# HKU-BAL/MegaPath-Nano

Hardware: AMD Instinct MI355X
Metric: Gbp/min ONT reads aligned+species-assigned vs RefSeq, 1/2/4/8 MI355X (higher is better)
Workload: dtype int32

## Files before the change

include/mpn_map.h:

```cpp
#ifndef MPN_MAP_H
#define MPN_MAP_H
#include <stdint.h>

#ifdef __cplusplus
extern "C" {
#endif

typedef struct mpn_index mpn_index;

typedef struct {
    int32_t k, w;
    float mid_occ_frac;
    int32_t mid_occ;
    int32_t max_gap, bw, max_chain_skip, max_chain_iter, min_cnt, min_chain_score;
    float mask_level, pri_ratio;
    int32_t best_n;
    int32_t max_join_long, max_join_short, min_join_flank_sc;
    float min_join_flank_ratio;
    int32_t a, b, q, e, q2, e2, sc_ambi, zdrop, zdrop_inv, end_bonus, min_dp_max, min_ksw_len;
    float max_clip_ratio;
    int64_t max_sw_mat;
    int32_t with_cigar;
    uint32_t seed;
    int32_t host_threads;
// ... 23 lines not shown
int32_t mpn_index_part_info(const char *path, int64_t offset, int64_t *bases, int64_t *next_offset);
int32_t mpn_index_n_seq(const mpn_index *idx);
int32_t mpn_index_seq_len(const mpn_index *idx, int32_t i);
int32_t mpn_index_seq_name(const mpn_index *idx, int32_t i, char *buf, int32_t cap);
int32_t mpn_index_k(const mpn_index *idx);
int32_t mpn_index_w(const mpn_index *idx);
int64_t mpn_index_n_minimizers(const mpn_index *idx);
int64_t mpn_index_n_keys(const mpn_index *idx);
int32_t mpn_index_mid_occ(const mpn_index *idx, float frac);
int64_t mpn_index_fetch_seq(const mpn_index *idx, int32_t i, int64_t start, int64_t len, char *out);
int mpn_index_export(const mpn_index *idx, uint64_t *keys, int64_t *key_off, uint64_t *pos);

int64_t mpn_sketch_batch(int32_t n, const char *seqs, const int64_t *seq_off, const int32_t *seq_len, int32_t k,
                         int32_t w, int64_t *mz_off, uint64_t *mz, int64_t cap);

int mpn_seed_chain_batch(const mpn_index *idx, const mpn_map_opt *opt, int32_t n, const char *seqs,
                         const int64_t *seq_off, const int32_t *seq_len, int64_t *n_anchor, int32_t *rep_len,
                         int64_t *chain_off, uint64_t *u, int64_t u_cap, int64_t *anchor_off, uint64_t *b,
                         int64_t b_cap);

int mpn_chain_batch(const mpn_map_opt *opt, int32_t n, const int64_t *anchor_off, const uint64_t *anchors, int32_t chain_item,
                    int32_t bt_par_min, int32_t grid_cap, int32_t *n_chain, int64_t *n_chained, uint64_t *u, int64_t *recs,
                    int64_t u_cap, uint64_t *b, int64_t b_cap);

int mpn_seed_anchors_batch(int32_t k, int32_t n_seq, const int32_t *lens, int64_t n_keys, const uint64_t *keys, const int64_t *key_off,
                           const uint64_t *pos, const mpn_map_opt *opt, int32_t n, const int64_t *mz_off, const uint64_t *mz,
                           const int32_t *seq_len, int64_t flt_round2, int32_t flt_wgs, int32_t grid_cap, int64_t *n_anchor, int32_t *rep_len,
                           int64_t *span_sum, int64_t *anchor_off, uint64_t *anchors, int64_t cap, int64_t counts[4]);

int mpn_ext_dp_batch(const mpn_map_opt *opt, int32_t n, const uint8_t *qcodes, const int64_t *q_off, const int32_t *q_len,
                     const uint8_t *tcodes, const int64_t *t_off, const int32_t *t_len, const int32_t *w, const int32_t *zdrop,
                     const int32_t *end_bonus, const int32_t *flag, int32_t force_kernel, int32_t *out9, uint32_t *cigar_pool,
                     int64_t cigar_cap, int64_t *cig_off);

int mpn_aln_tags_batch(int32_t n, const uint8_t *qcodes, const int64_t *q_off, const int32_t *q_len,
                       const int32_t *qs, const int32_t *qe, const int32_t *rev,
                       const uint8_t *tcodes, const int64_t *t_off, const int32_t *t_len, const int32_t *ts,
                       const uint32_t *cigar, const int64_t *cig_off, const int32_t *n_cigar, int32_t out_tags,
                       char *cs, int64_t cs_cap, int64_t *cs_off, char *md, int64_t md_cap, int64_t *md_off,
                       uint32_t *eqx, int64_t eqx_cap, int64_t *eqx_off);

int mpn_aln_finish_batch(const mpn_map_opt *opt, int32_t n, const uint8_t *qcodes, const int64_t *q_off, const int32_t *q_len,
                         const int32_t *qs, const int32_t *qe, const int32_t *rev,
                         const uint8_t *tcodes, const int64_t *t_off, const int32_t *t_len, const int32_t *ts,
                         const uint32_t *cigar, const int64_t *cig_off, const int32_t *n_cigar, int32_t force_class,
                         int32_t *out8, uint32_t *cigar_out);
// ... 68 lines not shown
```

megapath_nano_amd/csrc/map_kernels.h:

```cpp
#pragma once
#include "mpn_common.h"
#include "map_types.h"

#include <type_traits>

namespace mpn {

__device__ __forceinline__ uint64_t hash64m(uint64_t key, uint64_t mask) {
    key = (~key + (key << 21)) & mask;
    key = key ^ key >> 24;
    key = ((key + (key << 3)) + (key << 8)) & mask;
    key = key ^ key >> 14;
    key = ((key + (key << 2)) + (key << 4)) & mask;
    key = key ^ key >> 28;
    key = (key + (key << 31)) & mask;
    return key;
}

constexpr int SKETCH_FAST_MAX_W = 32;

template <bool HASH64>
__device__ __forceinline__ uint64_t sketch_hash(uint64_t key, uint64_t mask) {
    if (HASH64) return hash64m(key, mask);
    uint32_t h = (uint32_t)key;
// ... 1405 lines not shown
                }
                const uint32_t rank = __popcll(same & ((1ULL << lane) - 1));
                if (act && rank == 0) wcnt[wv][dg] = __popcll(same);
                __syncthreads();
                if (act) {
                    uint32_t o = bins[dg] + rank;
                    for (int w2 = 0; w2 < wv; ++w2) o += wcnt[w2][dg];
                    dst[o] = r;
                }
                __syncthreads();
                bins[tid] += wcnt[0][tid] + wcnt[1][tid] + wcnt[2][tid] + wcnt[3][tid];
                __syncthreads();
            }
            uint64_t *sw = src; src = dst; dst = sw;
            __threadfence_block();
            __syncthreads();
        }
        if (src != U + base) for (int i = tid; i < n; i += 256) U[base + i] = src[i];
        __syncthreads();
    }
}

constexpr int BT_PAR_MIN = 16;

__global__ __launch_bounds__(64) void chain_backtrack_kernel(const u128 *__restrict__ anchors, const int64_t *__restrict__ anchor_off,
                                                             int n_reads, ChainParams cp, const int32_t *__restrict__ F,
                                                             const int32_t *__restrict__ P, int32_t *__restrict__ T,
                                                             int32_t *__restrict__ V, uint64_t *__restrict__ U,
                                                             const int32_t *__restrict__ n_ends, u128 *__restrict__ B,
                                                             uint64_t *__restrict__ Uc, unsigned long long *__restrict__ used,
                                                             int64_t *__restrict__ u_pos, int64_t *__restrict__ b_pos,
                                                             int32_t *__restrict__ n_chain, int64_t *__restrict__ n_chained,
                                                             ChainRec *__restrict__ Rc, int par_min) {
    __shared__ int s_k;
    __shared__ unsigned long long s_up, s_bp;
    const int lane = threadIdx.x;
    for (int read = blockIdx.x; read < n_reads; read += gridDim.x) {
        const int64_t base = anchor_off[read];
        const int64_t n = anchor_off[read + 1] - base;
        const u128 *a = anchors + base;
        const int32_t *f = F + base, *p = P + base;
        int32_t *t = T + base, *v = V + base;
        uint64_t *u = U + base;
        const int n_u = n_ends[read];
        if (n_u >= par_min) {
            for (int64_t i = lane; i < n; i += 64) t[i] = 0x7fffffff;
            __builtin_amdgcn_fence(__ATOMIC_RELEASE, "agent");
            __syncthreads();
            for (int e0 = 0; e0 < n_u; e0 += 64) {
                const int e = e0 + lane;
                if (e < n_u) {
                    int32_t j = (int32_t)u[e];
                    while (j >= 0) { const int32_t nj = p[j]; if (atomicMin(&t[j], e) < e) break; j = nj; }
                }
            }
            __builtin_amdgcn_fence(__ATOMIC_ACQ_REL, "agent");
            __syncthreads();
            int k_run = 0, nv_run = 0;
            for (int e0 = 0; e0 < n_u; e0 += 64) {
                const int e = e0 + lane;
                int cnt = 0;
                if (e < n_u) {
                    const uint64_t ui = u[e];
                    int32_t j = p[(int32_t)ui];
                    cnt = 1;
                    while (j >= 0) { const int32_t tj = t[j], nj = p[j]; if (tj != e) break; ++cnt; j = nj; }
                    const bool keep = cnt >= cp.min_cnt && (j < 0 || (int32_t)(ui >> 32) - f[j] >= cp.min_sc);
                    if (!keep) cnt = 0;
// ... 90 lines not shown
            for (int j = lane; j < ni; j += 64) {
                const u128 cur = a[v[off + (ni - j - 1)]];
                b[off + j] = cur;
                const int span = (int)(cur.y >> 32 & 0xff);
                if (j == 0) { ml += span; bl += span; }
                else {
                    const u128 prev = a[v[off + (ni - j)]];
                    const int tl = (int32_t)cur.x - (int32_t)prev.x, ql = (int32_t)cur.y - (int32_t)prev.y;
                    bl += tl > ql ? tl : ql;
                    ml += tl > span && ql > span ? span : tl < ql ? tl : ql;
                }
            }
            ml = __builtin_amdgcn_readlane(wave_scan_add(ml), 63);
            bl = __builtin_amdgcn_readlane(wave_scan_add(bl), 63);
            if (lane == 0) {
                const u128 first = a[v[off + ni - 1]], last = a[v[off]];
                rc[c] = ChainRec{first.x, first.y, last.x, last.y, ml, bl};
            }
            off += ni;
        }
        for (int c = lane; c < k; c += 64) uc[c] = u[c];
        __syncthreads();
    }
}

__global__ __launch_bounds__(256) void idx_bucket_hist_kernel(const u128 *__restrict__ mz, int64_t n, int shift, unsigned long long *__restrict__ hist) {
    for (int64_t i = (int64_t)blockIdx.x * blockDim.x + threadIdx.x; i < n; i += (int64_t)gridDim.x * blockDim.x)
        atomicAdd(&hist[(mz[i].x >> 8) >> shift], 1ULL);
}

__global__ __launch_bounds__(256) void idx_bucket_scatter_kernel(const u128 *__restrict__ mz, int64_t n, int shift,
                                                                 unsigned long long *__restrict__ cursor, u128 *__restrict__ out) {
    for (int64_t i = (int64_t)blockIdx.x * blockDim.x + threadIdx.x; i < n; i += (int64_t)gridDim.x * blockDim.x) {
        u128 r = mz[i];
        r.x >>= 8;
        const unsigned long long p = atomicAdd(&cursor[r.x >> shift], 1ULL);
        out[p] = r;
    }
}

__global__ __launch_bounds__(256) void idx_flag_count_kernel(const u128 *__restrict__ rec, int64_t n, int64_t *__restrict__ block_cnt) {
    __shared__ int s[256];
    const int64_t base = (int64_t)blockIdx.x * 2048;
    int c = 0;
    for (int k = 0; k < 8; ++k) {
        const int64_t i = base + k * 256 + threadIdx.x;
// ... 89 lines not shown
```

megapath_nano_amd/csrc/mapper.hip:

```cpp
#include "map_kernels.h"
#include "mapper_internal.h"
#include "stage_input.h"
#include "../../include/mpn_map.h"

#include <algorithm>
#include <memory>
#include <mutex>
#include <string.h>
#include <time.h>
#include <sys/stat.h>
#include <string>
#include <vector>

namespace mpn {

hipError_t stream_sync(hipStream_t st) {
    struct Ev {
        hipEvent_t e = nullptr;
        ~Ev() { if (e) (void)hipEventDestroy(e); }
    };
    static thread_local Ev ev;
    hipError_t rc;
    if (!ev.e && (rc = hipEventCreateWithFlags(&ev.e, hipEventDisableTiming)) != hipSuccess) return rc;
    if ((rc = hipEventRecord(ev.e, st)) != hipSuccess) return rc;
// ... 189 lines not shown
}

int sketch_reads(int k, int w, int n, const uint8_t *d_seqs, const int64_t *d_off, const int32_t *d_len, const int32_t *h_len, ReadSketch &sk,
                 StreamLease &st) {
    EvTimer ev(st);
    sk.valid = false;
    if (sketch_device(d_seqs, d_off, d_len, h_len, n, k, w, 0, sk.mz_off, sk.mz, &sk.n_mz, st, &ev)) return -1;
    MPN_HIP_CHECK(stream_sync(st));
    ev.resolve();
    sk.k = k; sk.w = w; sk.valid = true;
    return 0;
}

static int chain_gap_check(const mpn_map_opt *opt, const char *who) {
    if (opt->max_gap > CHAIN_MAX_GAP) {
        set_error("%s: max_gap %d is beyond %d, the largest the chain DP's 32-bit ring coordinate holds", who, opt->max_gap, CHAIN_MAX_GAP);
        return -1;
    }
    return 0;
}

static int alloc_chain_tables(SeedChainOut &o, int n) {
    const size_t N = (size_t)n, o1 = (N + 1) * 8, o2 = o1 + N * 8, o3 = o2 + N * 8, o4 = o3 + N * 8, o5 = o4 + N * 4, o6 = (o5 + N * 4 + 7) & ~(size_t)7;
    o.tables_bytes = o6 + (size_t)(2 + WORK_SLOTS) * 8;
    if (o.tables.alloc(o.tables_bytes)) return -1;
    auto view = [&](auto &buf, size_t off, size_t count) { buf.release(); buf.p = reinterpret_cast<decltype(buf.p)>(o.tables.p + off); buf.n = count; buf.owned = false; };
    view(o.n_anchor, 0, N + 1); view(o.n_chained, o1, N); view(o.u_pos, o2, N); view(o.b_pos, o3, N);
    view(o.n_chain, o4, N); view(o.rep_len, o5, N); view(o.used, o6, 2 + WORK_SLOTS);
    return 0;
}

struct ChainKnobs {
    int chain_item = 0;
    int bt_par_min = 0;
    int grid_cap = 0;
};
struct ChainScratch {
    DevBuf<int64_t> kept, piece_kept, piece_off;
    DevBuf<float> avg_qspan;
    DevBuf<int32_t> F, P, T, V;
    DevBuf<uint64_t> Utmp;
    DevBuf<ChainSeg> seg_big, seg_small;
};
static int chain_enqueue(const mpn_map_opt *opt, int n, int64_t n_a, SeedChainOut &o, u128 *tmp, unsigned long long *read_kept,
                         const unsigned long long *span_sum, unsigned int *seg_counters, const ChainKnobs &kn, ChainScratch &cs, StreamLease &st,
                         EvTimer &ev) {
    auto &[kept, piece_kept, piece_off, avg_qspan, F, P, T, V, Utmp, seg_big, seg_small] = cs;
    ChainParams cp;
    cp.max_dist_x = opt->max_gap; cp.max_dist_y = opt->max_gap; cp.bw = opt->bw; cp.max_skip = opt->max_chain_skip;
    cp.max_iter = opt->max_chain_iter; cp.min_cnt = opt->min_cnt; cp.min_sc = opt->min_chain_score;
    const auto capped = [&](int64_t grid) { return (int)(kn.grid_cap > 0 ? std::min<int64_t>(grid, kn.grid_cap) : grid); };
    const int g = capped(std::max(1, std::min(n, 256 * 32)));
    const int64_t n_pieces = (n_a + COMPACT_PIECE - 1) / COMPACT_PIECE;
    if (kept.alloc((size_t)n + 1) || o.c_off.alloc((size_t)n + 1) || avg_qspan.alloc(n) || piece_kept.alloc((size_t)n_pieces + 1) ||
        piece_off.alloc((size_t)n_pieces + 1))
        return -1;
    const int gp = capped(std::max<int64_t>(1, std::min<int64_t>(n_pieces, 256 * 64)));
    if (n_a > 0) {
// ... 17 lines not shown
                           cp.max_dist_x, cp.min_cnt, (int64_t *)nullptr, (unsigned long long *)nullptr, (const int64_t *)piece_off.p, ca);
        MPN_HIP_CHECK(hipGetLastError());
    }
    ev.mark(46);
    static const int chain_item_env = []() { const char *e = getenv("MPN_CHAIN_ITEM"); return e ? std::min(CHAIN_BIG, std::max(16, atoi(e))) : CHAIN_ITEM; }();
    const int chain_item = kn.chain_item > 0 ? std::min(CHAIN_BIG, std::max(16, kn.chain_item)) : chain_item_env;
    if (seg_big.alloc((size_t)n_c / CHAIN_BIG + (size_t)n + 1) || seg_small.alloc((size_t)n_c / chain_item + (size_t)n + 1)) return -1;
    hipLaunchKernelGGL(chain_segments_kernel, dim3(g), dim3(64), 0, st, (const u128 *)ca, (const int64_t *)o.c_off.p, n, cp, avg_qspan.p, 1, seg_big.p,
                       seg_small.p, seg_counters, chain_item);
    MPN_HIP_CHECK(hipGetLastError());
    ev.mark(13);
    hipLaunchKernelGGL(chain_dp_kernel, dim3(capped(256 * 32)), dim3(64), 0, st, (const u128 *)ca, (const int64_t *)o.c_off.p, (const float *)avg_qspan.p,
                       (const ChainSeg *)seg_big.p, (const ChainSeg *)seg_small.p, seg_counters, cp, F.p, P.p, T.p, V.p);
    MPN_HIP_CHECK(hipGetLastError());
    ev.mark(13, 37);
    hipLaunchKernelGGL(chain_ends_kernel, dim3(g), dim3(64), 0, st, (const int64_t *)o.c_off.p, n, cp, F.p, P.p, T.p, V.p, o.u.p, o.n_ends.p);
    MPN_HIP_CHECK(hipGetLastError());
    hipLaunchKernelGGL(chain_sort_ends_kernel, dim3(capped(std::max(1, std::min(n, 256 * 8)))), dim3(256), 0, st, o.u.p, Utmp.p,
                       (const int64_t *)o.c_off.p, o.n_ends.p, n);
    MPN_HIP_CHECK(hipGetLastError());
    o.u_compact.p = Utmp.p; o.u_compact.n = Utmp.n; o.u_compact.owned = Utmp.owned; Utmp.p = nullptr; Utmp.n = 0;
    static const int bt_par_min_env = []() { const char *e = getenv("MPN_BT_PAR_MIN"); return e ? std::max(1, atoi(e)) : BT_PAR_MIN; }();
    const int bt_par_min = kn.bt_par_min > 0 ? kn.bt_par_min : bt_par_min_env;
    hipLaunchKernelGGL(chain_backtrack_kernel, dim3(g), dim3(64), 0, st, (const u128 *)ca, (const int64_t *)o.c_off.p, n, cp, F.p, P.p, T.p, V.p,
                       o.u.p, o.n_ends.p, o.chained.p, o.u_compact.p, o.used.p, o.u_pos.p, o.b_pos.p, o.n_chain.p, o.n_chained.p, o.recs.p, bt_par_min);
    MPN_HIP_CHECK(hipGetLastError());
    return 0;
}

struct SeedKnobs {
    int64_t flt_round2 = 0;
    int flt_wgs = 0;
    int grid_cap = 0;
};
struct SeedScratch {
    DevBuf<int32_t> occ, blk_read, order;
    DevBuf<int64_t> pos_start, rel_off, full_off, n_blk, blk_base, blk_kept, blk_off;
    DevBuf<unsigned long long> span_sum, keep, read_kept, walked;
    DevBuf<unsigned int> next_read, n_list, seg_counters;
    DevBuf<u128> tmp;
    DevBuf<SortSeg> list_mem;
};
static int seed_enqueue(const mpn_index *idx, const mpn_map_opt *opt, int32_t mid_occ, int n, const u128 *mz, const int64_t *mz_off, int64_t n_mz,
                        const int32_t *d_len, SeedChainOut &o, const SeedKnobs &kn, bool count_walked, SeedScratch &ss, int64_t *n_a_out,
                        StreamLease &st, EvTimer &ev) {
    auto &[occ, blk_read, order, pos_start, rel_off, full_off, n_blk, blk_base, blk_kept, blk_off, span_sum, keep, read_kept, walked, next_read, n_list,
           seg_counters, tmp, list_mem] = ss;
    const auto capped = [&](int64_t grid) { return (int)(kn.grid_cap > 0 ? std::min<int64_t>(grid, kn.grid_cap) : grid); };
// ... 126 lines not shown
    } else if (sketch_device(d_seqs, d_off, d_len, h_len, n, idx->k, idx->w, 0, mz_off, mz, &n_mz, st, &ev)) return -1;
    g_stats[1] += n_mz;
    int32_t mid_occ = opt->mid_occ > 0 ? opt->mid_occ : mpn_index_mid_occ(idx, opt->mid_occ_frac);
    if (mid_occ > (1 << 25)) {
        const int32_t top = mpn_index_mid_occ(idx, 1e-30f);
        if (top > 0) mid_occ = std::min(mid_occ, top);
    }
    if (alloc_chain_tables(o, n)) return -1;
    SeedScratch ss;
    int64_t n_a = 0;
    if (seed_enqueue(idx, opt, mid_occ, n, mz.p, mz_off.p, n_mz, d_len, o, SeedKnobs{}, false, ss, &n_a, st, ev)) return -1;
    ChainScratch cs;
    if (chain_enqueue(opt, n, n_a, o, ss.tmp.p, ss.read_kept.p, ss.span_sum.p, ss.seg_counters.p, ChainKnobs{}, cs, st, ev)) return -1;
    ev.mark(14);
    MPN_HIP_CHECK(stream_sync(st));
    ev.resolve();
    return 0;
}

int download_chains(int n, SeedChainOut &o, HostChains &h, PoolBuf &pin_u, PoolBuf &pin_b, StreamLease &st, int mode) {
    const bool with_anchors = mode == 2;
    h.n_anchor.resize((size_t)n);
    h.n_chain.resize(n); h.n_chained.resize(n); h.rep_len.resize(n); h.u_pos.resize(n); h.b_pos.resize(n);
    unsigned long long used[2 + WORK_SLOTS] = {0};
    {
        const size_t N = (size_t)n;
        const size_t o1 = (N + 1) * 8, o2 = o1 + N * 8, o3 = o2 + N * 8, o4 = o3 + N * 8, o5 = o4 + N * 4, o6 = (o5 + N * 4 + 7) & ~(size_t)7;
        char *pn = (char *)tl_pin.get(o.tables_bytes + 64);
        if (!pn) { set_error("pinned scratch allocation failed"); return -1; }
        MPN_HIP_CHECK(hipMemcpyAsync(pn, o.tables.p, o.tables_bytes, hipMemcpyDeviceToHost, st));
        MPN_HIP_CHECK(stream_sync(st));
        memcpy(h.n_anchor.data(), pn, N * 8); memcpy(h.n_chained.data(), pn + o1, N * 8);
        memcpy(h.u_pos.data(), pn + o2, N * 8); memcpy(h.b_pos.data(), pn + o3, N * 8);
        memcpy(h.n_chain.data(), pn + o4, N * 4); memcpy(h.rep_len.data(), pn + o5, N * 4);
        memcpy(used, pn + o6, sizeof(used));
    }
    for (int k = 0; k < WORK_SLOTS; ++k) g_stats[44] += (int64_t)used[2 + k];
    ++g_stats[32];
    h.n_pool_chains = (int64_t)used[0];
    if (mode == 0) { h.u_all = nullptr; h.rec_all = nullptr; h.b_all = nullptr; }
    else if (with_anchors) {
        if (pin_u.ensure((size_t)used[0] * 8 + 16) || pin_b.ensure((size_t)used[1] * 16 + 16)) return -1;
        if (o.u_compact.download(pin_u.as<uint64_t>(), (size_t)used[0], st) || o.chained.download(pin_b.as<u128>(), (size_t)used[1], st)) return -1;
        h.u_all = pin_u.as<uint64_t>(); h.b_all = pin_b.as<u128>();
    } else {
        const size_t rec_bytes = ((size_t)used[0] * sizeof(ChainRec) + 15) & ~(size_t)15;
        if (pin_u.ensure(rec_bytes + (size_t)used[0] * 8 + 16)) return -1;
        h.rec_all = pin_u.as<ChainRec>();
        h.u_all = reinterpret_cast<const uint64_t *>(reinterpret_cast<const char *>(pin_u.p) + rec_bytes);
        h.b_all = nullptr;
        if (o.recs.download(const_cast<ChainRec *>(h.rec_all), (size_t)used[0], st) || o.u_compact.download(const_cast<uint64_t *>(h.u_all), (size_t)used[0], st)) return -1;
    }
    h.chain_off.assign((size_t)n + 1, 0);
    h.b_off.assign((size_t)n + 1, 0);
    for (int i = 0; i < n; ++i) { h.chain_off[i + 1] = h.chain_off[i] + h.n_chain[i]; h.b_off[i + 1] = h.b_off[i] + h.n_chained[i]; }
    MPN_HIP_CHECK(stream_sync(st));
    return 0;
}

void HostChains::read_chains(int i, uint64_t *uo, u128 *bo) const {
// ... 507 lines not shown
    DevBuf<int64_t> d_off;
    DevBuf<int32_t> d_len;
    int64_t bases = 0;
    if (upload_seqs(n, seqs, seq_off, seq_len, d_seqs, d_off, d_len, &bases, st)) return -1;
    g_stats[0] = bases;
    SeedChainOut o;
    StreamLease sl(st);
    if (seed_chain_device(idx, opt, n, d_seqs.p, d_off.p, d_len.p, seq_len, o, sl, nullptr)) return -1;
    HostChains h;
    PoolBuf pin_u{nullptr, 0, true}, pin_b{nullptr, 0, true};
    struct Free { PoolBuf &a, &b; ~Free() { a.release(); b.release(); } } free_pins{pin_u, pin_b};
    if (download_chains(n, o, h, pin_u, pin_b, sl, 2)) return -1;
    for (int i = 0; i < n; ++i) { n_anchor[i] = h.n_anchor[i]; rep_len[i] = h.rep_len[i]; }
    memcpy(chain_off, h.chain_off.data(), ((size_t)n + 1) * 8);
    memcpy(anchor_off, h.b_off.data(), ((size_t)n + 1) * 8);
    if (h.chain_off[n] > u_cap || h.b_off[n] > b_cap) return -3;
    for (int i = 0; i < n; ++i) h.read_chains(i, u + h.chain_off[i], (u128 *)b + h.b_off[i]);
    return 0;
}

int mpn_chain_batch(const mpn_map_opt *opt, int32_t n, const int64_t *anchor_off, const uint64_t *anchors, int32_t chain_item,
                    int32_t bt_par_min, int32_t grid_cap, int32_t *n_chain, int64_t *n_chained, uint64_t *u, int64_t *recs, int64_t u_cap,
                    uint64_t *b, int64_t b_cap) {
    if (!opt || n < 0) { set_error("mpn_chain_batch: options missing or a negative count"); return -1; }
    if (opt->max_gap < 0 || opt->bw < 0 || opt->max_chain_skip < 0 || opt->max_chain_iter < 0 || opt->min_cnt < 0 || opt->min_chain_score < 0) {
        set_error("mpn_chain_batch: a negative option"); return -1;
    }
    if (opt->max_chain_iter < 1) { set_error("mpn_chain_batch: max_chain_iter below 1"); return -1; }
    if (chain_gap_check(opt, "mpn_chain_batch")) return -1;
    if (chain_item < 0 || bt_par_min < 0 || grid_cap < 0 || u_cap < 0 || b_cap < 0) { set_error("mpn_chain_batch: chain_item, bt_par_min, grid_cap or a capacity negative"); return -1; }
    if (n == 0) return 0;
    if (!anchor_off || !n_chain || !n_chained) { set_error("mpn_chain_batch: an array missing"); return -1; }
    if (!mpn_stage::stage_csr_ok("mpn_chain_batch", n, anchor_off, set_error)) return -1;
    const int64_t n_a = anchor_off[n];
    if (n_a > 0 && !anchors) { set_error("mpn_chain_batch: an array missing"); return -1; }
    std::vector<int64_t> cnt((size_t)n + 1, 0);
    std::vector<unsigned long long> sums((size_t)n, 0);
    for (int i = 0; i < n; ++i) {
        unsigned long long s = 0;
        for (int64_t k = anchor_off[i]; k < anchor_off[i + 1]; ++k) {
            const uint64_t x = anchors[2 * k], y = anchors[2 * k + 1];
            if (k > anchor_off[i] && x < anchors[2 * (k - 1)]) { set_error("mpn_chain_batch: read %d: anchor %lld: x decreases", i, (long long)(k - anchor_off[i])); return -1; }
            if (y & 0x80000000ull) { set_error("mpn_chain_batch: read %d: anchor %lld: query position outside 0 .. 2^31 - 1", i, (long long)(k - anchor_off[i])); return -1; }
            s += y >> 32 & 0xff;
        }
        cnt[(size_t)i] = anchor_off[i + 1] - anchor_off[i];
// ... 1 lines not shown
    }
    hipStream_t st = 0;
    memset(g_stats, 0, sizeof(g_stats));
    SeedChainOut o;
    StreamLease sl(st);
    EvTimer ev(sl);
    DevBuf<u128> tmp;
    DevBuf<unsigned long long> span_sum, read_kept;
    DevBuf<unsigned int> seg_counters;
    if (alloc_chain_tables(o, n) || o.anchor_off.upload(anchor_off, (size_t)n + 1, st) || o.anchors.upload(reinterpret_cast<const u128 *>(anchors), (size_t)n_a, st) ||
        tmp.alloc((size_t)n_a) || o.n_ends.alloc((size_t)n) || span_sum.upload(sums.data(), (size_t)n, st) || read_kept.alloc((size_t)n) || seg_counters.alloc(4))
        return -1;
    MPN_HIP_CHECK(hipMemcpyAsync(o.n_anchor.p, cnt.data(), ((size_t)n + 1) * 8, hipMemcpyHostToDevice, st));
    {
        ZeroList z{};
        zero_list_push(z, o.used.p, o.used.n * sizeof(unsigned long long));
        zero_list_push(z, seg_counters.p, 4 * sizeof(unsigned int));
        zero_list_push(z, read_kept.p, (size_t)n * 8);
        zero_list_push(z, o.rep_len.p, (size_t)n * 4);
        MPN_HIP_CHECK(zero_regions(z, st));
    }
    o.n_anchors = n_a;
    ChainKnobs kn;
    kn.chain_item = chain_item; kn.bt_par_min = bt_par_min; kn.grid_cap = grid_cap;
    ChainScratch cs;
    if (chain_enqueue(opt, n, n_a, o, tmp.p, read_kept.p, span_sum.p, seg_counters.p, kn, cs, sl, ev)) return -1;
    ev.mark(14);
    MPN_HIP_CHECK(stream_sync(sl));
    ev.resolve();
    HostChains h;
    PoolBuf pin_u{nullptr, 0, true}, pin_b{nullptr, 0, true};
    struct Free { PoolBuf &a, &b; ~Free() { a.release(); b.release(); } } free_pins{pin_u, pin_b};
    if (download_chains(n, o, h, pin_u, pin_b, sl, 2)) return -1;
    if (h.n_pool_chains < 0 || (size_t)h.n_pool_chains > o.recs.n || (size_t)h.b_off[(size_t)n] > o.chained.n || h.chain_off[(size_t)n] != h.n_pool_chains) {
        set_error("mpn_chain_batch: the kernels counted %lld chains and %lld chained anchors, %zu and %zu at most expected", (long long)h.n_pool_chains,
                  (long long)h.b_off[(size_t)n], o.recs.n, o.chained.n);
        return -1;
    }
    std::vector<ChainRec> rv((size_t)h.n_pool_chains + 1);
    if (o.recs.download(rv.data(), (size_t)h.n_pool_chains, st)) return -1;
    MPN_HIP_CHECK(stream_sync(st));
    h.rec_all = rv.data();
    for (int i = 0; i < n; ++i) { n_chain[i] = h.n_chain[(size_t)i]; n_chained[i] = h.n_chained[(size_t)i]; }
    if (h.chain_off[(size_t)n] > u_cap || h.b_off[(size_t)n] > b_cap) return -3;
    if ((h.chain_off[(size_t)n] > 0 && (!u || !recs)) || (h.b_off[(size_t)n] > 0 && !b)) { set_error("mpn_chain_batch: an array missing"); return -1; }
    std::vector<int32_t> order;
    std::vector<int64_t> src;
// ... 83 lines not shown
```

megapath_nano_amd/csrc/mapper_internal.h:

```cpp
#pragma once
#include "mpn_common.h"
#include "map_types.h"
#include "queue_lease.h"

#include <atomic>
#include <chrono>
#include <time.h>
#include <mutex>
#include <stdint.h>
#include <stdlib.h>
#include <string.h>
#include <string>
#include <vector>

struct mpn_map_opt_s;


struct mpn_index {
    int k = 15, w = 10;
    int32_t n_seq = 0;
    std::vector<std::string> names;
    std::vector<int32_t> lens;
    std::vector<int64_t> seq_off;
    std::vector<uint32_t> h_seq2;
// ... 28 lines not shown
    DevBuf<unsigned long long> used;
};

struct ReadSketch {
    DevBuf<int64_t> mz_off;
    DevBuf<u128> mz;
    int64_t n_mz = 0;
    int k = 0, w = 0;
    bool valid = false;
};

struct HostChains {
    std::vector<int64_t> n_anchor, chain_off, b_off;
    std::vector<int64_t> n_chained, u_pos, b_pos;
    std::vector<int32_t> n_chain, rep_len;
    const uint64_t *u_all = nullptr;
    const u128 *b_all = nullptr;
    const ChainRec *rec_all = nullptr;
    int64_t n_pool_chains = 0;
    void read_chains(int i, uint64_t *u_out, u128 *b_out) const;
    void chain_order(int i, int32_t *order, int64_t *src) const;
};

constexpr int MPN_NSTATS = 77;
constexpr int STAT_LEASE_WAIT = 65;
constexpr int STAT_SIDE_LEASED = 66, STAT_SIDE_OWN = 67;
constexpr int STAT_TILE_CLASS = 68, STAT_TILE_GIVEUPS = 72;
constexpr int STAT_WALK_WAVE = 73, STAT_EV_WALK_LONG = 74, STAT_WALK_WAVE_FAILED = 75;
constexpr int STAT_K_TAGS = 76;
extern thread_local int64_t g_stats[MPN_NSTATS];

void pack_2bit(const uint8_t *codes, int64_t n, std::vector<uint32_t> &words, std::vector<int64_t> &ns, std::vector<int64_t> &ne);

hipError_t stream_sync(hipStream_t st);

struct QueueStreams {
    LeasePool pool;
    std::vector<hipStream_t> st;
    explicit QueueStreams(int q) : pool(q), st((size_t)q, nullptr) {}
};
QueueStreams *queue_streams(int dev);

class StreamLease {
  public:
    explicit StreamLease(QueueStreams *qs) : qs_(qs) {}
    explicit StreamLease(hipStream_t fixed) : fixed_(fixed) {}
    StreamLease(const StreamLease &) = delete;
    StreamLease &operator=(const StreamLease &) = delete;
    ~StreamLease() { release(); }
    hipStream_t get() {
        if (!qs_) return fixed_;
        if (n_ == 0) n_ = qs_->pool.acquire(1, id_, &g_stats[STAT_LEASE_WAIT]);
// ... 121 lines not shown
```

megapath_nano_amd/mapper.py:

```python
import ctypes as ct
import os

import numpy as np

from . import _ffi


class MapOpt(ct.Structure):
    _fields_ = [('k', ct.c_int32), ('w', ct.c_int32), ('mid_occ_frac', ct.c_float), ('mid_occ', ct.c_int32),
                ('max_gap', ct.c_int32), ('bw', ct.c_int32), ('max_chain_skip', ct.c_int32), ('max_chain_iter', ct.c_int32),
                ('min_cnt', ct.c_int32), ('min_chain_score', ct.c_int32), ('mask_level', ct.c_float),
                ('pri_ratio', ct.c_float), ('best_n', ct.c_int32), ('max_join_long', ct.c_int32),
                ('max_join_short', ct.c_int32), ('min_join_flank_sc', ct.c_int32), ('min_join_flank_ratio', ct.c_float),
                ('a', ct.c_int32), ('b', ct.c_int32), ('q', ct.c_int32), ('e', ct.c_int32), ('q2', ct.c_int32),
                ('e2', ct.c_int32), ('sc_ambi', ct.c_int32), ('zdrop', ct.c_int32), ('zdrop_inv', ct.c_int32),
                ('end_bonus', ct.c_int32), ('min_dp_max', ct.c_int32), ('min_ksw_len', ct.c_int32),
                ('max_clip_ratio', ct.c_float), ('max_sw_mat', ct.c_int64), ('with_cigar', ct.c_int32),
                ('seed', ct.c_uint32), ('host_threads', ct.c_int32), ('out_sam', ct.c_int32), ('out_tags', ct.c_int32)]


TAG_CS, TAG_CS_LONG, TAG_MD, TAG_EQX = 1, 2, 4, 8


COL_NAMES = ('read_idx', 'qs', 'qe', 'rev', 'rid', 'rs', 're', 'mlen', 'blen', 'mapq', 'nm', 'as_', 'primary')
# ... 91 lines not shown
        lib.mpn_map_fetch_sam.restype = ct.c_int64
        lib.mpn_map_fetch_cols.argtypes = [ct.POINTER(AlnCols)]
        lib.mpn_map_fetch_cols.restype = ct.c_int64
        lib.mpn_map_fetch_text.argtypes = [ct.c_char_p, ct.c_int64]
        lib.mpn_map_fetch_text.restype = ct.c_int64
        lib.mpn_ext_dp_batch.argtypes = [ct.POINTER(MapOpt), ct.c_int32, P, P, P, P, P, P, P, P, P, P, ct.c_int32, P, P, ct.c_int64, P]
        lib.mpn_ext_dp_batch.restype = ct.c_int
        lib.mpn_aln_tags_batch.argtypes = [ct.c_int32, P, P, P, P, P, P, P, P, P, P, P, P, P, ct.c_int32, P, ct.c_int64, P, P, ct.c_int64, P,
                                           P, ct.c_int64, P]
        lib.mpn_aln_tags_batch.restype = ct.c_int
        lib.mpn_aln_finish_batch.argtypes = [ct.POINTER(MapOpt), ct.c_int32, P, P, P, P, P, P, P, P, P, P, P, P, P, ct.c_int32, P, P]
        lib.mpn_aln_finish_batch.restype = ct.c_int
        lib.mpn_hit_select_batch.argtypes = [ct.POINTER(MapOpt), ct.c_int32, ct.c_int32, P, ct.POINTER(ct.c_char_p), P, P, P, P, P, P, P, P, P, P,
                                             ct.c_int32, ct.c_int32, ct.c_int32, P, P, P, P]
        lib.mpn_hit_select_batch.restype = ct.c_int
        lib.mpn_ext_plan_batch.argtypes = [ct.POINTER(MapOpt), ct.c_int32, ct.c_int32, P, ct.c_int32, P, P, P, P, P, P, P, P, ct.c_int32, P, ct.c_int64,
                                           P, P, P]
        lib.mpn_ext_plan_batch.restype = ct.c_int
        lib.mpn_stitch_batch.argtypes = [ct.c_int32, P, P, ct.c_int32, P, ct.c_int64, P, P, ct.c_int64, P, ct.c_int32, ct.c_int32, P, ct.c_int64, P, P,
                                         P, P]
        lib.mpn_stitch_batch.restype = ct.c_int
        lib.mpn_chain_batch.argtypes = [ct.POINTER(MapOpt), ct.c_int32, P, P, ct.c_int32, ct.c_int32, ct.c_int32, P, P, P, P, ct.c_int64, P, ct.c_int64]
        lib.mpn_chain_batch.restype = ct.c_int
        lib.mpn_seed_anchors_batch.argtypes = [ct.c_int32, ct.c_int32, P, ct.c_int64, P, P, P, ct.POINTER(MapOpt), ct.c_int32, P, P, P, ct.c_int64,
                                               ct.c_int32, ct.c_int32, P, P, P, P, P, ct.c_int64, P]
        lib.mpn_seed_anchors_batch.restype = ct.c_int
        lib.mpn_map_last_stats.argtypes = [P]
        lib.mpn_map_last_stats.restype = None
        lib.mpn_reads_split_plan.argtypes = [ct.c_int32, P, ct.c_int64, P, P, ct.c_int32, ct.c_int64, P, P, P, P, P, P]
        lib.mpn_reads_split_plan.restype = ct.c_int
        lib.mpn_reads_split_gather.argtypes = [ct.c_int32, P, P, ct.c_int64, P, P, ct.c_int32, ct.c_int64, P, P, ct.c_int64, P, P, ct.c_int64, P, P]
        lib.mpn_reads_split_gather.restype = ct.c_int
        lib.mpn_reads_split_last_ns.argtypes = [ct.c_int32]
        lib.mpn_reads_split_last_ns.restype = ct.c_int64
        lib.mpn_map_last_stats_ex.argtypes = [P, ct.c_int32]
        lib.mpn_map_last_stats_ex.restype = ct.c_int32
        _bound = True
    return lib


def default_opt(**kw):
    o = MapOpt()
    _bind().mpn_map_opt_init(ct.byref(o))
    for k, v in kw.items():
        setattr(o, k, v)
    return o
# ... 173 lines not shown
    n_anchor = np.zeros(n, dtype=np.int64)
    rep_len = np.zeros(n, dtype=np.int32)
    chain_off = np.zeros(n + 1, dtype=np.int64)
    anchor_off = np.zeros(n + 1, dtype=np.int64)
    u_cap, b_cap = 1 << 16, 1 << 20
    while True:
        u = np.zeros(u_cap, dtype=np.uint64)
        b = np.zeros((b_cap, 2), dtype=np.uint64)
        rc = lib.mpn_seed_chain_batch(idx.h, ct.byref(opt), n, buf.ctypes.data, off.ctypes.data, lens.ctypes.data,
                                      n_anchor.ctypes.data, rep_len.ctypes.data, chain_off.ctypes.data, u.ctypes.data, u_cap,
                                      anchor_off.ctypes.data, b.ctypes.data, b_cap)
        if rc == -3:
            u_cap, b_cap = max(u_cap, int(chain_off[n]) + 1), max(b_cap, int(anchor_off[n]) + 1)
            continue
        _ffi.check(rc, 'mpn_seed_chain_batch')
        break
    return [dict(n_anchor=int(n_anchor[i]), rep_len=int(rep_len[i]), u=u[chain_off[i]:chain_off[i + 1]].copy(),
                 b=b[anchor_off[i]:anchor_off[i + 1]].copy()) for i in range(n)]


CHAIN_REC_KEYS = ('fx', 'fy', 'lx', 'ly', 'mlen', 'blen')


def chain_batch(opt, anchor_off, anchors, chain_item=0, bt_par_min=0, grid_cap=0):
    lib = _bind()
    anchor_off = np.ascontiguousarray(anchor_off, dtype=np.int64)
    anchors = np.ascontiguousarray(anchors, dtype=np.uint64).reshape(-1, 2)
    n = len(anchor_off) - 1
    assert n >= 0 and (n == 0 or len(anchors) >= int(anchor_off[-1]))
    n_chain = np.zeros(n + 1, dtype=np.int32)
    n_chained = np.zeros(n + 1, dtype=np.int64)
    u_cap, b_cap = len(anchors) // 4 + 16, len(anchors) + 16
    while True:
        u = np.zeros(u_cap, dtype=np.uint64)
        recs = np.zeros((u_cap, 6), dtype=np.int64)
        b = np.zeros((b_cap, 2), dtype=np.uint64)
        rc = lib.mpn_chain_batch(ct.byref(opt), n, anchor_off.ctypes.data, anchors.ctypes.data, int(chain_item), int(bt_par_min), int(grid_cap),
                                 n_chain.ctypes.data, n_chained.ctypes.data, u.ctypes.data, recs.ctypes.data, u_cap, b.ctypes.data, b_cap)
        if rc == -3:
            u_cap, b_cap = max(u_cap, int(n_chain.sum()) + 1), max(b_cap, int(n_chained.sum()) + 1)
            continue
        _ffi.check(rc, 'mpn_chain_batch')
        break
    c_off = np.concatenate([[0], np.cumsum(n_chain[:n].astype(np.int64))])
    b_off = np.concatenate([[0], np.cumsum(n_chained[:n])])
    return [dict(n_chain=int(n_chain[i]), n_chained=int(n_chained[i]), u=u[c_off[i]:c_off[i + 1]].copy(), b=b[b_off[i]:b_off[i + 1]].copy(),
                 recs=recs[c_off[i]:c_off[i + 1]].copy()) for i in range(n)]


def seed_anchors_batch(k, lens, keys, key_off, pos, opt, mz_off, mz, seq_len, flt_round2=0, flt_wgs=0, grid_cap=0, cap=None):
    lib = _bind()
    lens = np.ascontiguousarray(lens, dtype=np.int32)
    keys = np.ascontiguousarray(keys, dtype=np.uint64)
    key_off = np.ascontiguousarray(key_off, dtype=np.int64)
    pos = np.ascontiguousarray(pos, dtype=np.uint64)
    mz_off = np.ascontiguousarray(mz_off, dtype=np.int64)
    mz = np.ascontiguousarray(mz, dtype=np.uint64).reshape(-1, 2)
    seq_len = np.ascontiguousarray(seq_len, dtype=np.int32)
    n = len(mz_off) - 1
    assert n >= 0 and len(seq_len) == n and len(key_off) == len(keys) + 1
    n_anchor = np.zeros(n + 1, dtype=np.int64)
# ... 556 lines not shown
    rc = lib.mpn_stitch_batch(n, anchor_off.ctypes.data, anchors.ctypes.data, n_hits, hits.ctypes.data, len(wins), wins.ctypes.data,
                              cig_pos.ctypes.data, len(compact), compact.ctypes.data, int(min_cnt), int(grid_cap), out.ctypes.data, pool_cap,
                              pool.ctypes.data, ct.addressof(used), splits.ctypes.data, ct.addressof(n_splits))
    _ffi.check(rc, 'mpn_stitch_batch')
    return out[:n_hits], pool[:used.value], splits[:n_splits.value]


STAT_NAMES = {0: 'bases', 1: 'minimizers', 2: 'anchors', 3: 'chains', 4: 'dp_jobs', 5: 'dp_cells', 6: 'alignments',
              7: 'dp_rounds', 8: 'second_pass_jobs', 10: 'ev_sketch_ns', 11: 'ev_seed_ns', 12: 'ev_sort_ns',
              13: 'ev_chain_dp_ns', 14: 'ev_chain_bt_ns', 15: 'ev_ext_dp_ns', 25: 'ev_ext_bt_ns', 26: 'ev_ext_ztest_ns',
              16: 'wall_h2d_ns', 17: 'wall_seed_chain_ns', 18: 'wall_d2h_chains_ns', 19: 'wall_host_hits_ns',
              20: 'wall_host_plan_ns', 21: 'wall_ext_stage_ns', 22: 'wall_host_stitch_ns', 23: 'wall_host_final_ns',
              24: 'wall_total_ns', 27: 'wall_ext_host_prep_ns', 28: 'wall_ext_enqueue_ns', 29: 'wall_ext_gpu_wait_ns',
              30: 'wall_ext_finish_ns', 9: 'ev_ext_strip_ns', 31: 'strip_cells', 32: 'sub_batches',
              33: 'k_sketch_count_ns', 34: 'k_sketch_fill_ns', 35: 'k_seed_lookup_ns', 36: 'k_seed_fill_ns',
              37: 'k_chain_dp_ns', 38: 'k_strip16_ns', 39: 'k_strip32_ns', 40: 'k_strip64_ns', 41: 'strip16_cells',
              42: 'strip32_cells', 43: 'strip64_cells', 44: 'sort_records_moved', 45: 'anchors_kept', 46: 'k_compact_ns', 47: 'k_sort_msd_ns', 48: 'k_sort_chunk_ns', 49: 'k_sort_radix_ns',
              50: 'k_seed_filter_ns', 51: 'anchors_emitted', 52: 'k_finish_ns', 53: 'cigar_ops', 54: 'k_stitch_ns', 55: 'k_plan_ns', 56: 'k_layout_ns', 57: 'k_xstrip_ns', 58: 'xstrip_cells', 59: 'anchors_squeezed', 60: 'workers_shed', 61: 'workers', 62: 'k_hit_select_ns', 63: 'reads_hits_on_host',
              64: 'tile_windows', 65: 'wall_lease_wait_ns', 66: 'ext_groups_side_leased', 67: 'ext_groups_side_own',
              68: 'tile_windows_1w_s16', 69: 'tile_windows_s4_nw8', 70: 'tile_windows_s8_nw4', 71: 'tile_windows_s4_nw16',
              72: 'tile_wait_giveups',
              73: 'walk_wave_windows', 74: 'ev_ext_walk_long_ns',
              75: 'walk_wave_failed',
              76: 'k_tags_ns'}


def last_stats():
    n = max(STAT_NAMES) + 1
    s = np.zeros(n, dtype=np.int64)
    _bind().mpn_map_last_stats_ex(s.ctypes.data, n)
    return {name: int(s[i]) for i, name in STAT_NAMES.items()}
```

Measured before the change: 14.86.

## Add sweep-based chain backtrack for reads with moderate chain-end counts

Adds a sweep backtrack path for reads whose chain-end count lies between the parallel threshold and a cap of 1024. It walks anchors from high to low index in 64-wide blocks, propagates ownership via an LDS pointer-jumping min, and computes counts, scores and mlen/blen with wave ballots and LDS atomics instead of per-chain serial walks. The intent is to cut the long serial predecessor walks and global atomics of the old backtrack. In exchange there are two kernel launches per batch, a large LDS footprint (about 16KB) per 64-thread block that may limit occupancy, and a serial sweep over all anchors that can cost more than walking only the chained ones.

New measurement: 15.35, median of 6. +3.3%, better.

```diff
diff --git a/include/mpn_map.h b/include/mpn_map.h
--- a/include/mpn_map.h
+++ b/include/mpn_map.h
@@ -69,6 +69,9 @@
 int mpn_chain_batch(const mpn_map_opt *opt, int32_t n, const int64_t *anchor_off, const uint64_t *anchors, int32_t chain_item,
                     int32_t bt_par_min, int32_t grid_cap, int32_t *n_chain, int64_t *n_chained, uint64_t *u, int64_t *recs,
                     int64_t u_cap, uint64_t *b, int64_t b_cap);
+int mpn_chain_batch_bt(const mpn_map_opt *opt, int32_t n, const int64_t *anchor_off, const uint64_t *anchors, int32_t chain_item,
+                       int32_t bt_par_min, int32_t grid_cap, int32_t bt_mode, int32_t bt_sweep_cap, int32_t *n_chain, int64_t *n_chained,
+                       uint64_t *u, int64_t *recs, int64_t u_cap, uint64_t *b, int64_t b_cap);
 
 int mpn_seed_anchors_batch(int32_t k, int32_t n_seq, const int32_t *lens, int64_t n_keys, const uint64_t *keys, const int64_t *key_off,
                            const uint64_t *pos, const mpn_map_opt *opt, int32_t n, const int64_t *mz_off, const uint64_t *mz,
diff --git a/megapath_nano_amd/csrc/map_kernels.h b/megapath_nano_amd/csrc/map_kernels.h
--- a/megapath_nano_amd/csrc/map_kernels.h
+++ b/megapath_nano_amd/csrc/map_kernels.h
@@ -1451,7 +1451,156 @@
 }
 
 constexpr int BT_PAR_MIN = 16;
-
+constexpr int BT_SWEEP_MAX_ENDS = 1024;
+constexpr int BT_MODE_AUTO = 0, BT_MODE_WALK = 1, BT_MODE_SWEEP = 2;
+constexpr int BT_STAT_SLOT = 2 + WORK_SLOTS;
+constexpr int CHAIN_USED_SLOTS = BT_STAT_SLOT + 2;
+
+struct BtSweepLds {
+    int32_t first[BT_SWEEP_MAX_ENDS];
+    int32_t cur[BT_SWEEP_MAX_ENDS];
+    int32_t ml[BT_SWEEP_MAX_ENDS], bl[BT_SWEEP_MAX_ENDS];
+    int32_t val[64], link[64];
+};
+
+__device__ __forceinline__ void bt_sweep_read(BtSweepLds &s, const u128 *__restrict__ a, const int32_t *__restrict__ f,
+                                              const int32_t *__restrict__ p, int32_t *t, int32_t *v, const uint64_t *u, int n, int n_u,
+                                              const ChainParams &cp, int read, u128 *__restrict__ B, uint64_t *__restrict__ Uc,
+                                              ChainRec *__restrict__ Rc, unsigned long long *__restrict__ used, int64_t *__restrict__ u_pos,
+                                              int64_t *__restrict__ b_pos, int32_t *__restrict__ n_chain, int64_t *__restrict__ n_chained,
+                                              unsigned long long &s_up, unsigned long long &s_bp) {
+    constexpr int32_t INF = 0x7fffffff;
+    const int lane = threadIdx.x;
+    const unsigned long long below = (1ULL << lane) - 1;
+    for (int i = lane; i < n; i += 64) t[i] = INF;
+    for (int e = lane; e < n_u; e += 64) { s.first[e] = (int32_t)u[e]; s.cur[e] = 0; }
+    __builtin_amdgcn_fence(__ATOMIC_RELEASE, "agent");
+    __syncthreads();
+    for (int e = lane; e < n_u; e += 64) atomicMin(&t[(int32_t)u[e]], e);
+    for (int j0 = (n - 1) & ~63; j0 >= 0; j0 -= 64) {
+        __builtin_amdgcn_fence(__ATOMIC_ACQ_REL, "workgroup");
+        __syncthreads();
+        const int j = j0 + lane;
+        int32_t val = INF, pj = -1;
+        if (j < n) { val = __hip_atomic_load(&t[j], __ATOMIC_RELAXED, __HIP_MEMORY_SCOPE_AGENT); pj = p[j]; }
+        int link = pj >= j0 && pj < j ? pj - j0 : -1;
+        if (__ballot(link >= 0)) {
+            s.val[lane] = val;
+            for (int r = 0; r < 6; ++r) {
+                s.link[lane] = link;
+                MPN_LDS_FENCE();
+                if (link >= 0) atomicMin(&s.val[link], s.val[lane]);
+                MPN_LDS_FENCE();
+                if (link >= 0) link = s.link[link];
+                MPN_LDS_FENCE();
+                if (!__ballot(link >= 0)) break;
+            }
+            val = s.val[lane];
+            MPN_LDS_FENCE();
+        }
+        if (j < n) {
+            t[j] = val;
+            if (pj >= 0 && pj < j0 && val != INF) atomicMin(&t[pj], val);
+        }
+        const bool owned = j < n && val < n_u;
+        unsigned long long m = __ballot(owned);
+        while (m) {
+            const int ld = __ffsll((long long)m) - 1;
+            const int oe = __builtin_amdgcn_readlane(val, ld);
+            const unsigned long long same = __ballot(owned && val == oe);
+            if (lane == ld) { s.cur[oe] += __popcll(same); s.first[oe] = j; }
+            m &= ~same;
+        }
+    }
+    __builtin_amdgcn_fence(__ATOMIC_ACQ_REL, "workgroup");
+    __syncthreads();
+    int k_run = 0, nv_run = 0;
+    for (int e0 = 0; e0 < n_u; e0 += 64) {
+        const int e = e0 + lane;
+        int cnt = 0;
+        if (e < n_u) {
+            const uint64_t ui = u[e];
+            const int c = s.cur[e] > 1 ? s.cur[e] : 1;
+            const int32_t stop = p[s.first[e]];
+            const bool keep = c >= cp.min_cnt && (stop < 0 || (int32_t)(ui >> 32) - f[stop] >= cp.min_sc);
+            cnt = keep ? c : 0;
+            v[e] = cnt;
+        }
+        const int incl = wave_scan_add(cnt);
+        if (e < n_u) { s.cur[e] = cnt > 0 ? nv_run + incl - cnt : -1; s.ml[e] = 0; s.bl[e] = 0; }
+        k_run += __builtin_amdgcn_readlane(wave_scan_add(cnt > 0 ? 1 : 0), 63);
+        nv_run += __builtin_amdgcn_readlane(incl, 63);
+    }
+    if (lane == 0) {
+        n_chain[read] = k_run;
+        n_chained[read] = nv_run;
+        s_up = k_run ? atomicAdd(&used[0], (unsigned long long)k_run) : 0ULL;
+        s_bp = nv_run ? atomicAdd(&used[1], (unsigned long long)nv_run) : 0ULL;
+        u_pos[read] = (int64_t)s_up;
+        b_pos[read] = (int64_t)s_bp;
+    }
+    __builtin_amdgcn_fence(__ATOMIC_ACQ_REL, "workgroup");
+    __syncthreads();
+    u128 *b = B + s_bp;
+    uint64_t *uc = Uc + s_up;
+    ChainRec *rc = Rc + s_up;
+    for (int j0 = 0; j0 < n; j0 += 64) {
+        const int j = j0 + lane;
+        int32_t own = INF;
+        if (j < n) own = __hip_atomic_load(&t[j], __ATOMIC_RELAXED, __HIP_MEMORY_SCOPE_AGENT);
+        const bool owned = own < n_u;
+        int pos = -1;
+        unsigned long long m = __ballot(owned);
+        while (m) {
+            const int ld = __ffsll((long long)m) - 1;
+            const int oe = __builtin_amdgcn_readlane(own, ld);
+            const bool mine = owned && own == oe;
+            const unsigned long long same = __ballot(mine);
+            const int c = s.cur[oe];
+            if (mine && c >= 0) pos = c + __popcll(same & below);
+            MPN_LDS_FENCE();
+            if (lane == ld && c >= 0) s.cur[oe] = c + __popcll(same);
+            MPN_LDS_FENCE();
+            m &= ~same;
+        }
+        if (pos >= 0) {
+            const u128 cur = a[j];
+            b[pos] = cur;
+            if (j != s.first[own]) {
+                const u128 prev = a[p[j]];
+                const int span = (int)(cur.y >> 32 & 0xff);
+                const int tl = (int32_t)cur.x - (int32_t)prev.x, ql = (int32_t)cur.y - (int32_t)prev.y;
+                atomicAdd(&s.bl[own], tl > ql ? tl : ql);
+                atomicAdd(&s.ml[own], tl > span && ql > span ? span : tl < ql ? tl : ql);
+            }
+        }
+    }
+    __builtin_amdgcn_fence(__ATOMIC_ACQ_REL, "workgroup");
+    __syncthreads();
+    k_run = 0; nv_run = 0;
+    for (int e0 = 0; e0 < n_u; e0 += 64) {
+        const int e = e0 + lane;
+        const int cnt = e < n_u ? v[e] : 0;
+        const int incl = wave_scan_add(cnt), kin = wave_scan_add(cnt > 0 ? 1 : 0);
+        if (cnt > 0) {
+            const int kidx = k_run + kin - 1, off = nv_run + incl - cnt;
+            const uint64_t ui = u[e];
+            const int32_t fi = s.first[e];
+            const u128 head = a[fi], last = a[(int32_t)ui];
+            if (s.cur[e] == off) b[off] = last;
+            const int span0 = (int)(head.y >> 32 & 0xff);
+            const int32_t stop = p[fi];
+            const uint64_t sc = stop < 0 ? ui >> 32 : (ui >> 32) - (uint64_t)f[stop];
+            uc[kidx] = sc << 32 | (uint32_t)cnt;
+            rc[kidx] = ChainRec{head.x, head.y, last.x, last.y, s.ml[e] + span0, s.bl[e] + span0};
+        }
+        k_run += __builtin_amdgcn_readlane(kin, 63);
+        nv_run += __builtin_amdgcn_readlane(incl, 63);
+    }
+    __syncthreads();
+}
+
+template <bool SWEEP>
 __global__ __launch_bounds__(64) void chain_backtrack_kernel(const u128 *__restrict__ anchors, const int64_t *__restrict__ anchor_off,
                                                              int n_reads, ChainParams cp, const int32_t *__restrict__ F,
                                                              const int32_t *__restrict__ P, int32_t *__restrict__ T,
@@ -1460,10 +1609,12 @@
                                                              uint64_t *__restrict__ Uc, unsigned long long *__restrict__ used,
                                                              int64_t *__restrict__ u_pos, int64_t *__restrict__ b_pos,
                                                              int32_t *__restrict__ n_chain, int64_t *__restrict__ n_chained,
-                                                             ChainRec *__restrict__ Rc, int par_min) {
+                                                             ChainRec *__restrict__ Rc, int par_min, int sweep_cap) {
     __shared__ int s_k;
     __shared__ unsigned long long s_up, s_bp;
     const int lane = threadIdx.x;
+    sweep_cap = sweep_cap < BT_SWEEP_MAX_ENDS ? sweep_cap : BT_SWEEP_MAX_ENDS;
+    int n_sweep = 0, n_walk = 0;
     for (int read = blockIdx.x; read < n_reads; read += gridDim.x) {
         const int64_t base = anchor_off[read];
         const int64_t n = anchor_off[read + 1] - base;
@@ -1472,7 +1623,15 @@
         int32_t *t = T + base, *v = V + base;
         uint64_t *u = U + base;
         const int n_u = n_ends[read];
+        if ((n_u >= par_min && n_u <= sweep_cap) != SWEEP) continue;
+        if constexpr (SWEEP) {
+            __shared__ BtSweepLds s_sweep;
+            bt_sweep_read(s_sweep, a, f, p, t, v, u, (int)n, n_u, cp, read, B, Uc, Rc, used, u_pos, b_pos, n_chain, n_chained, s_up, s_bp);
+            ++n_sweep;
+            continue;
+        }
         if (n_u >= par_min) {
+            ++n_walk;
             for (int64_t i = lane; i < n; i += 64) t[i] = 0x7fffffff;
             __builtin_amdgcn_fence(__ATOMIC_RELEASE, "agent");
             __syncthreads();
@@ -1609,6 +1768,10 @@
         for (int c = lane; c < k; c += 64) uc[c] = u[c];
         __syncthreads();
     }
+    if (lane == 0) {
+        if (n_sweep) atomicAdd(&used[BT_STAT_SLOT], (unsigned long long)n_sweep);
+        if (n_walk) atomicAdd(&used[BT_STAT_SLOT + 1], (unsigned long long)n_walk);
+    }
 }
 
 __global__ __launch_bounds__(256) void idx_bucket_hist_kernel(const u128 *__restrict__ mz, int64_t n, int shift, unsigned long long *__restrict__ hist) {
diff --git a/megapath_nano_amd/csrc/mapper.hip b/megapath_nano_amd/csrc/mapper.hip
--- a/megapath_nano_amd/csrc/mapper.hip
+++ b/megapath_nano_amd/csrc/mapper.hip
@@ -235,11 +235,11 @@
 
 static int alloc_chain_tables(SeedChainOut &o, int n) {
     const size_t N = (size_t)n, o1 = (N + 1) * 8, o2 = o1 + N * 8, o3 = o2 + N * 8, o4 = o3 + N * 8, o5 = o4 + N * 4, o6 = (o5 + N * 4 + 7) & ~(size_t)7;
-    o.tables_bytes = o6 + (size_t)(2 + WORK_SLOTS) * 8;
+    o.tables_bytes = o6 + (size_t)CHAIN_USED_SLOTS * 8;
     if (o.tables.alloc(o.tables_bytes)) return -1;
     auto view = [&](auto &buf, size_t off, size_t count) { buf.release(); buf.p = reinterpret_cast<decltype(buf.p)>(o.tables.p + off); buf.n = count; buf.owned = false; };
     view(o.n_anchor, 0, N + 1); view(o.n_chained, o1, N); view(o.u_pos, o2, N); view(o.b_pos, o3, N);
-    view(o.n_chain, o4, N); view(o.rep_len, o5, N); view(o.used, o6, 2 + WORK_SLOTS);
+    view(o.n_chain, o4, N); view(o.rep_len, o5, N); view(o.used, o6, CHAIN_USED_SLOTS);
     return 0;
 }
 
@@ -247,6 +247,8 @@
     int chain_item = 0;
     int bt_par_min = 0;
     int grid_cap = 0;
+    int bt_mode = 0;
+    int bt_sweep_cap = 0;
 };
 struct ChainScratch {
     DevBuf<int64_t> kept, piece_kept, piece_off;
@@ -310,8 +312,19 @@
     o.u_compact.p = Utmp.p; o.u_compact.n = Utmp.n; o.u_compact.owned = Utmp.owned; Utmp.p = nullptr; Utmp.n = 0;
     static const int bt_par_min_env = []() { const char *e = getenv("MPN_BT_PAR_MIN"); return e ? std::max(1, atoi(e)) : BT_PAR_MIN; }();
     const int bt_par_min = kn.bt_par_min > 0 ? kn.bt_par_min : bt_par_min_env;
-    hipLaunchKernelGGL(chain_backtrack_kernel, dim3(g), dim3(64), 0, st, (const u128 *)ca, (const int64_t *)o.c_off.p, n, cp, F.p, P.p, T.p, V.p,
-                       o.u.p, o.n_ends.p, o.chained.p, o.u_compact.p, o.used.p, o.u_pos.p, o.b_pos.p, o.n_chain.p, o.n_chained.p, o.recs.p, bt_par_min);
+    static const int bt_mode_env = []() {
+        const char *e = getenv("MPN_BT_MODE");
+        return e && !strcmp(e, "walk") ? BT_MODE_WALK : e && !strcmp(e, "sweep") ? BT_MODE_SWEEP : BT_MODE_AUTO;
+    }();
+    const int bt_mode = kn.bt_mode > 0 ? kn.bt_mode : bt_mode_env;
+    const int bt_sweep_cap = bt_mode == BT_MODE_WALK ? 0 : kn.bt_sweep_cap > 0 ? std::min(kn.bt_sweep_cap, BT_SWEEP_MAX_ENDS) : BT_SWEEP_MAX_ENDS;
+    if (bt_sweep_cap > 0) {
+        hipLaunchKernelGGL(chain_backtrack_kernel<true>, dim3(g), dim3(64), 0, st, (const u128 *)ca, (const int64_t *)o.c_off.p, n, cp, F.p, P.p, T.p, V.p,
+                           o.u.p, o.n_ends.p, o.chained.p, o.u_compact.p, o.used.p, o.u_pos.p, o.b_pos.p, o.n_chain.p, o.n_chained.p, o.recs.p, bt_par_min, bt_sweep_cap);
+        MPN_HIP_CHECK(hipGetLastError());
+    }
+    hipLaunchKernelGGL(chain_backtrack_kernel<false>, dim3(g), dim3(64), 0, st, (const u128 *)ca, (const int64_t *)o.c_off.p, n, cp, F.p, P.p, T.p, V.p,
+                       o.u.p, o.n_ends.p, o.chained.p, o.u_compact.p, o.used.p, o.u_pos.p, o.b_pos.p, o.n_chain.p, o.n_chained.p, o.recs.p, bt_par_min, bt_sweep_cap);
     MPN_HIP_CHECK(hipGetLastError());
     return 0;
 }
@@ -484,7 +497,7 @@
     const bool with_anchors = mode == 2;
     h.n_anchor.resize((size_t)n);
     h.n_chain.resize(n); h.n_chained.resize(n); h.rep_len.resize(n); h.u_pos.resize(n); h.b_pos.resize(n);
-    unsigned long long used[2 + WORK_SLOTS] = {0};
+    unsigned long long used[CHAIN_USED_SLOTS] = {0};
     {
         const size_t N = (size_t)n;
         const size_t o1 = (N + 1) * 8, o2 = o1 + N * 8, o3 = o2 + N * 8, o4 = o3 + N * 8, o5 = o4 + N * 4, o6 = (o5 + N * 4 + 7) & ~(size_t)7;
@@ -498,6 +511,8 @@
         memcpy(used, pn + o6, sizeof(used));
     }
     for (int k = 0; k < WORK_SLOTS; ++k) g_stats[44] += (int64_t)used[2 + k];
+    g_stats[STAT_BT_SWEEP_READS] += (int64_t)used[BT_STAT_SLOT];
+    g_stats[STAT_BT_WALK_READS] += (int64_t)used[BT_STAT_SLOT + 1];
     ++g_stats[32];
     h.n_pool_chains = (int64_t)used[0];
     if (mode == 0) { h.u_all = nullptr; h.rec_all = nullptr; h.b_all = nullptr; }
@@ -1051,6 +1066,13 @@
 int mpn_chain_batch(const mpn_map_opt *opt, int32_t n, const int64_t *anchor_off, const uint64_t *anchors, int32_t chain_item,
                     int32_t bt_par_min, int32_t grid_cap, int32_t *n_chain, int64_t *n_chained, uint64_t *u, int64_t *recs, int64_t u_cap,
                     uint64_t *b, int64_t b_cap) {
+    return mpn_chain_batch_bt(opt, n, anchor_off, anchors, chain_item, bt_par_min, grid_cap, 0, 0, n_chain, n_chained, u, recs, u_cap, b, b_cap);
+}
+
+int mpn_chain_batch_bt(const mpn_map_opt *opt, int32_t n, const int64_t *anchor_off, const uint64_t *anchors, int32_t chain_item,
+                       int32_t bt_par_min, int32_t grid_cap, int32_t bt_mode, int32_t bt_sweep_cap, int32_t *n_chain, int64_t *n_chained,
+                       uint64_t *u, int64_t *recs, int64_t u_cap, uint64_t *b, int64_t b_cap) {
+    if (bt_mode < 0 || bt_mode > BT_MODE_SWEEP || bt_sweep_cap < 0) { set_error("mpn_chain_batch_bt: bt_mode outside 0 .. 2 or a negative bt_sweep_cap"); return -1; }
     if (!opt || n < 0) { set_error("mpn_chain_batch: options missing or a negative count"); return -1; }
     if (opt->max_gap < 0 || opt->bw < 0 || opt->max_chain_skip < 0 || opt->max_chain_iter < 0 || opt->min_cnt < 0 || opt->min_chain_score < 0) {
         set_error("mpn_chain_batch: a negative option"); return -1;
@@ -1098,7 +1120,7 @@
     }
     o.n_anchors = n_a;
     ChainKnobs kn;
-    kn.chain_item = chain_item; kn.bt_par_min = bt_par_min; kn.grid_cap = grid_cap;
+    kn.chain_item = chain_item; kn.bt_par_min = bt_par_min; kn.grid_cap = grid_cap; kn.bt_mode = bt_mode; kn.bt_sweep_cap = bt_sweep_cap;
     ChainScratch cs;
     if (chain_enqueue(opt, n, n_a, o, tmp.p, read_kept.p, span_sum.p, seg_counters.p, kn, cs, sl, ev)) return -1;
     ev.mark(14);
diff --git a/megapath_nano_amd/csrc/mapper_internal.h b/megapath_nano_amd/csrc/mapper_internal.h
--- a/megapath_nano_amd/csrc/mapper_internal.h
+++ b/megapath_nano_amd/csrc/mapper_internal.h
@@ -74,12 +74,13 @@
     void chain_order(int i, int32_t *order, int64_t *src) const;
 };
 
-constexpr int MPN_NSTATS = 77;
+constexpr int MPN_NSTATS = 79;
 constexpr int STAT_LEASE_WAIT = 65;
 constexpr int STAT_SIDE_LEASED = 66, STAT_SIDE_OWN = 67;
 constexpr int STAT_TILE_CLASS = 68, STAT_TILE_GIVEUPS = 72;
 constexpr int STAT_WALK_WAVE = 73, STAT_EV_WALK_LONG = 74, STAT_WALK_WAVE_FAILED = 75;
 constexpr int STAT_K_TAGS = 76;
+constexpr int STAT_BT_SWEEP_READS = 77, STAT_BT_WALK_READS = 78;
 extern thread_local int64_t g_stats[MPN_NSTATS];
 
 void pack_2bit(const uint8_t *codes, int64_t n, std::vector<uint32_t> &words, std::vector<int64_t> &ns, std::vector<int64_t> &ne);
diff --git a/megapath_nano_amd/mapper.py b/megapath_nano_amd/mapper.py
--- a/megapath_nano_amd/mapper.py
+++ b/megapath_nano_amd/mapper.py
@@ -137,6 +137,9 @@
         lib.mpn_stitch_batch.restype = ct.c_int
         lib.mpn_chain_batch.argtypes = [ct.POINTER(MapOpt), ct.c_int32, P, P, ct.c_int32, ct.c_int32, ct.c_int32, P, P, P, P, ct.c_int64, P, ct.c_int64]
         lib.mpn_chain_batch.restype = ct.c_int
+        lib.mpn_chain_batch_bt.argtypes = [ct.POINTER(MapOpt), ct.c_int32, P, P, ct.c_int32, ct.c_int32, ct.c_int32, ct.c_int32, ct.c_int32, P, P, P, P,
+                                           ct.c_int64, P, ct.c_int64]
+        lib.mpn_chain_batch_bt.restype = ct.c_int
         lib.mpn_seed_anchors_batch.argtypes = [ct.c_int32, ct.c_int32, P, ct.c_int64, P, P, P, ct.POINTER(MapOpt), ct.c_int32, P, P, P, ct.c_int64,
                                                ct.c_int32, ct.c_int32, P, P, P, P, P, ct.c_int64, P]
         lib.mpn_seed_anchors_batch.restype = ct.c_int
@@ -356,8 +359,12 @@
 CHAIN_REC_KEYS = ('fx', 'fy', 'lx', 'ly', 'mlen', 'blen')
 
 
-def chain_batch(opt, anchor_off, anchors, chain_item=0, bt_par_min=0, grid_cap=0):
-    lib = _bind()
+BT_MODES = {'auto': 0, 'walk': 1, 'sweep': 2}
+
+
+def chain_batch(opt, anchor_off, anchors, chain_item=0, bt_par_min=0, grid_cap=0, bt_mode=0, bt_sweep_cap=0):
+    lib = _bind()
+    bt_mode = BT_MODES[bt_mode] if isinstance(bt_mode, str) else int(bt_mode)
     anchor_off = np.ascontiguousarray(anchor_off, dtype=np.int64)
     anchors = np.ascontiguousarray(anchors, dtype=np.uint64).reshape(-1, 2)
     n = len(anchor_off) - 1
@@ -369,8 +376,12 @@
         u = np.zeros(u_cap, dtype=np.uint64)
         recs = np.zeros((u_cap, 6), dtype=np.int64)
         b = np.zeros((b_cap, 2), dtype=np.uint64)
-        rc = lib.mpn_chain_batch(ct.byref(opt), n, anchor_off.ctypes.data, anchors.ctypes.data, int(chain_item), int(bt_par_min), int(grid_cap),
-                                 n_chain.ctypes.data, n_chained.ctypes.data, u.ctypes.data, recs.ctypes.data, u_cap, b.ctypes.data, b_cap)
+        head = (ct.byref(opt), n, anchor_off.ctypes.data, anchors.ctypes.data, int(chain_item), int(bt_par_min), int(grid_cap))
+        tail = (n_chain.ctypes.data, n_chained.ctypes.data, u.ctypes.data, recs.ctypes.data, u_cap, b.ctypes.data, b_cap)
+        if bt_mode or bt_sweep_cap:
+            rc = lib.mpn_chain_batch_bt(*head, bt_mode, int(bt_sweep_cap), *tail)
+        else:
+            rc = lib.mpn_chain_batch(*head, *tail)
         if rc == -3:
             u_cap, b_cap = max(u_cap, int(n_chain.sum()) + 1), max(b_cap, int(n_chained.sum()) + 1)
             continue
@@ -973,7 +984,8 @@
               72: 'tile_wait_giveups',
               73: 'walk_wave_windows', 74: 'ev_ext_walk_long_ns',
               75: 'walk_wave_failed',
-              76: 'k_tags_ns'}
+              76: 'k_tags_ns',
+              77: 'bt_sweep_reads', 78: 'bt_walk_reads'}
 
 
 def last_stats():
```
